# libjxl/jxl-rs

Measured on AMD Instinct MI355X. Metric: megapixels/sec decoded (8K VarDCT d1 reconstruction: dequant+CfL+IDCT+LF smoothing+Gaborish+EPF), higher is better.
Workload: dtype f32

## Files before the change

### jxl_rs_amd/csrc/k_vardct.hip

```cpp
#include <algorithm>
#include <atomic>

#include "k_vardct_common.h"

#ifndef JXLH_NT_COEF
#define JXLH_NT_COEF true
#endif
#ifndef JXLH_NT_K1_STORE
#define JXLH_NT_K1_STORE true
#endif
namespace jxlh {
namespace {

constexpr int kScanGroups = 4;
constexpr int kScanThreads = kScanGroups * kThreads;
template <bool STRIP, bool ENT = false, bool ROUTE = false>
__global__ __launch_bounds__(kScanThreads) void k1_scan(const FrameDev f, const WorkLists wl, const int group_row0,
                                                         int* __restrict__ error_flag,
                                                         const int* __restrict__ group_list, const int ngroups,
                                                         int* __restrict__ next_counts) {
  constexpr int kPairs = (kNumClasses + 1) / 2;
  __shared__ int s_wave_sum[kScanGroups][kWaves];
  __shared__ uint32_t s_wcls[kScanGroups][kWaves][kPairs];
  __shared__ int s_count[kScanGroups][kNumClasses], s_base[kScanGroups][kNumClasses];
  __shared__ int s_route[ROUTE ? kScanGroups : 1];
  __shared__ int s_tmode[kScanGroups][16];
  __shared__ uint64_t s_pref[ENT ? kScanGroups : 1][ENT ? kSlotsPerRun + 1 : 1];
  __shared__ uint64_t s_wpref[ENT ? kScanGroups : 1][kWaves];
  if constexpr (STRIP) {
    if (threadIdx.x < kScanGroups * 16) s_tmode[threadIdx.x / 16][threadIdx.x % 16] = 0;
    if (blockIdx.x == 0)
      for (int i = threadIdx.x; i < f.strip_nflags; i += kScanThreads) f.strip_flags[i] = 0;
    __syncthreads();
  }
  if (blockIdx.x == 0 && threadIdx.x < kCountLines) next_counts[threadIdx.x * kCountPitch] = 0;
  const int sub = threadIdx.x / kThreads, tid = threadIdx.x % kThreads, lane = tid & 63, wave = tid >> 6;
  const int gi = blockIdx.x * kScanGroups + sub;
  const bool live = gi < ngroups;
  const int group = !live ? 0 : group_list ? group_list[gi] : group_row0 * f.xgroups + gi;
  const int bx0 = (group % f.xgroups) * kGroupBlocks, by0 = (group / f.xgroups) * kGroupBlocks;
  const int bw = live ? min(kGroupBlocks, f.xblocks - bx0) : 0, bh = live ? min(kGroupBlocks, f.yblocks - by0) : 0;
  int sizes[4], types[4], rq4[4], local = 0;
  const int by = tid >> 3, bx4 = (tid & 7) * 4;
  const int gby = min(by0 + by, f.yblocks - 1);
  uint8_t raw4[4];
#pragma unroll
  for (int i = 0; i < 4; i++) {
    const size_t at = (size_t)gby * f.xblocks + min(bx0 + bx4 + i, f.xblocks - 1);
    raw4[i] = f.transform_map[at];
    rq4[i] = f.raw_quant[at];
  }
  const int ci = (gby / kColorTileBlocks) * f.cmap_stride + min(bx0 + bx4, f.xblocks - 1) / kColorTileBlocks;
  const uint32_t cc = (uint32_t)(uint8_t)f.ytox[ci] | (uint32_t)(uint8_t)f.ytob[ci] << 8;
  uint32_t cw[3] = {0u, 0u, 0u};
  uint2 run[3] = {make_uint2(0u, 0u), make_uint2(0u, 0u), make_uint2(0u, 0u)};
  bool dense_route = false;
  if constexpr (ENT) {
    if constexpr (ROUTE) {
      dense_route = live && f.group_route[group] != 0;
      if (tid == 0) s_route[sub] = dense_route ? 1 : 0;
    }
    if (live && !dense_route) {
#pragma unroll
      for (int c = 0; c < 3; c++) {
        cw[c] = *reinterpret_cast<const uint32_t*>(f.se_counts + ((size_t)group * 3 + c) * kSlotsPerRun + 4 * tid);
        run[c] = f.se_runs[group * 3 + c];
      }
    }
  }
#pragma unroll
  for (int i = 0; i < 4; i++) {
    const int bx = bx4 + i;
    const uint8_t raw = (bx < bw && by < bh) ? raw4[i] : 0;
    const int type = raw & 127;
    int sz = 0;
    if (raw >= 128) {
      if (type < JXLH_NUM_TRANSFORMS) {
        const int cx = 1 << log2_covered_x_reg(type), cy = 1 << log2_covered_y_reg(type);
        sz = cx * cy;
        if (f.subsampled && sz > 1) atomicExch(error_flag, JXLH_ERR_INVALID_BLOCK_SIZE);
        if (bx + cx > bw || by + cy > bh) {
          atomicExch(error_flag, JXLH_ERR_BLOCK_OUT_OF_BOUNDS);
          sz = 0;
        }
        if constexpr (STRIP) {
          const bool closed = (bx & 3) + cx <= 4 && (by & 3) + cy <= 4 && class_of_type_reg(type) < kClsSpecial;
          if (sz == 0 || f.subsampled) {
            for (int k = 0; k < 16; k++) atomicOr(&s_tmode[sub][k], 1);
          } else if (!closed) {
            for (int ty = by >> 3; ty <= (by + cy - 1) >> 3; ty++)
              for (int tx = bx >> 3; tx <= (bx + cx - 1) >> 3; tx++) atomicOr(&s_tmode[sub][ty * 4 + tx], 1);
          }
        }
      } else {
        atomicExch(error_flag, JXLH_ERR_INVALID_TRANSFORM);
        if constexpr (STRIP)
          for (int k = 0; k < 16; k++) atomicOr(&s_tmode[sub][k], 1);
      }
    }
    sizes[i] = sz;
    types[i] = type;
    local += sz;
  }
  int incl = local;
#pragma unroll
  for (int d = 1; d < 64; d <<= 1) {
    const int n = __shfl_up(incl, d, 64);
    if (lane >= d) incl += n;
  }
  if (lane == 63) s_wave_sum[sub][wave] = incl;
  uint64_t pmine = 0, pincl = 0;
  if constexpr (ENT) {
    auto bytes = [](uint32_t w) { return (uint64_t)((w & 0xffu) + ((w >> 8) & 0xffu) + ((w >> 16) & 0xffu) + (w >> 24)); };
    pmine = bytes(cw[0]) | bytes(cw[1]) << 17 | bytes(cw[2]) << 34;
    pincl = pmine;
#pragma unroll
    for (int d = 1; d < 64; d <<= 1) {
      const uint32_t lo = (uint32_t)__shfl_up((int)(uint32_t)pincl, d, 64), hi = (uint32_t)__shfl_up((int)(uint32_t)(pincl >> 32), d, 64);
      if (lane >= d) pincl += (uint64_t)lo | (uint64_t)hi << 32;
    }
    if (lane == 63) s_wpref[sub][wave] = pincl;
  }
  int slot[4], cls4[4];
  bool strip_tile = false;
  if constexpr (STRIP) {
    __syncthreads();
    strip_tile = s_tmode[sub][(by >> 3) * 4 + (bx4 >> 3)] == 0;
  }
  uint32_t mine[kPairs], excl[kPairs];
#pragma unroll
  for (int w = 0; w < kPairs; w++) mine[w] = 0;
#pragma unroll
  for (int i = 0; i < 4; i++) {
    const int cls = sizes[i] > 0 && !strip_tile ? class_of_type_reg(types[i]) : -1;
    cls4[i] = cls;
    slot[i] = 0;
    const int sh = (cls & 1) * 16;
#pragma unroll
    for (int w = 0; w < kPairs; w++) {
      if ((cls >> 1) == w) {
        slot[i] = (int)((mine[w] >> sh) & 0xffffu);
        mine[w] += 1u << sh;
      }
    }
  }
#pragma unroll
  for (int w = 0; w < kPairs; w++) {
    uint32_t inc = mine[w];
#pragma unroll
    for (int d = 1; d < 64; d <<= 1) {
      const uint32_t n = (uint32_t)__shfl_up((int)inc, d, 64);
      if (lane >= d) inc += n;
    }
    excl[w] = inc - mine[w];
    if (lane == 63) s_wcls[sub][wave][w] = inc;
  }
  __syncthreads();
  if constexpr (ENT) {
    uint64_t base = pincl - pmine;
#pragma unroll
    for (int v = 0; v < kWaves; v++)
      if (v < wave) base += s_wpref[sub][v];
    uint64_t* P = s_pref[sub] + 4 * tid;
#pragma unroll
// ... 226 lines not shown
      }
    };
    EX x = shfl_up(packed, 1);
    if (j == 0) x = 0;
#pragma unroll
    for (int d = 1; d < NS; d <<= 1) {
      const EX y = shfl_up(x, d);
      if (j >= d) x += y;
    }
    if (j < NS) s_excl[b * NS + j] = x;
  }
}
template <class S, class EX>
__device__ __forceinline__ int entry_pos(const EX* __restrict__ s_excl, int b, int ch, uint32_t e, uint32_t r) {
  constexpr int NS = S::N / 64, B = excl_bits<EX>();
  int sidx = 0;
  if constexpr (NS > 1) {
#pragma unroll
    for (int step = NS / 2; step >= 1; step >>= 1) {
      const uint32_t v = (uint32_t)(s_excl[b * NS + sidx + step] >> (B * ch)) & ((1u << B) - 1u);
      if (r >= v) sidx += step;
    }
  }
  return sidx * 64 + (int)(e & 63u);
}
template <class S>
__device__ __forceinline__ void zero_tile(int* __restrict__ ibuf, int lane) {
  constexpr int kWords = S::NB * S::SM;
  if constexpr (kWords % 4 == 0) {
    for (int i = lane * 4; i < kWords; i += 256) *reinterpret_cast<int4*>(ibuf + i) = make_int4(0, 0, 0, 0);
  } else {
    for (int i = lane; i < kWords; i += 64) ibuf[i] = 0;
  }
}

template <class S, int D, class EX, bool HELD = true>
__device__ __forceinline__ void entries_stage_channel(const FrameDev& f, int ch, float* __restrict__ buf,
                                                      const EX* __restrict__ s_excl, int lane, const EntLane<D>& sl,
                                                      const BlockInfo* __restrict__ binfo = nullptr, int nb = 0) {
  int* ibuf = reinterpret_cast<int*>(buf);
  zero_tile<S>(ibuf, lane);
  wave_sync();
  constexpr int LPB = 64 / S::NB;
  const int b = lane / LPB, j = lane % LPB;
  auto add = [&](uint32_t e, uint32_t r) {
    atomicAdd(&ibuf[m_addr<S>(b, entry_pos<S, EX>(s_excl, b, ch, e, r))], (int)(e << 16) >> 22);
  };
  constexpr int DH = HELD ? D : 0;
  uint32_t i0 = 0, i1 = 0;
  if constexpr (HELD) {
    i0 = sl.i0[ch];
    i1 = sl.i1[ch];
  } else if (b < nb) {
    i0 = binfo[b].e0[ch] + j;
    i1 = binfo[b].e0[ch] + binfo[b].en[ch];
  }
#pragma unroll
  for (int k = 0; k < DH; k++)
    if (i0 + k * LPB < i1) add(sl.e[ch][k], (uint32_t)(j + k * LPB));
  constexpr int U = 4;
  uint32_t r = (uint32_t)(j + DH * LPB), i = i0 + DH * LPB;
  while (__any(i < i1)) {
    uint32_t ev[U];
#pragma unroll
    for (int u = 0; u < U; u++) ev[u] = i + u * LPB < i1 ? (uint32_t)f.se_entries[i + u * LPB] : 0u;
#pragma unroll
    for (int u = 0; u < U; u++)
      if (i + u * LPB < i1) add(ev[u], r + u * LPB);
    i += U * LPB;
    r += U * LPB;
  }
  wave_sync();
}

template <int D>
struct EntDirect {
  uint32_t ad[3][D];
};
constexpr uint32_t kNoEntry = 0xffffffffu;
constexpr int kClaimed = (int)0x80000000;

template <class S, int CH, int D>
__device__ __forceinline__ void direct_stage_channel(const FrameDev& f, float* __restrict__ buf, int lane,
                                                     const EntDirect<D>& ed, const float* __restrict__ table, int tsize,
                                                     float sdy, float cc, const AdjTable* __restrict__ adj,
                                                     float (&dyw)[D], uint32_t& ywin) {
  int* ibuf = reinterpret_cast<int*>(buf);
  constexpr int LPB = 64 / S::NB;
  const int b = lane / LPB;
  float w[D];
#pragma unroll
  for (int k = 0; k < D; k++) w[k] = ed.ad[CH][k] != kNoEntry ? table[CH * tsize + (int)(ed.ad[CH][k] & 0xffffu)] : 0.0f;
  zero_tile<S>(ibuf, lane);
  wave_sync();
  int at[D];
#pragma unroll
  for (int k = 0; k < D; k++) {
    at[k] = m_addr<S>(b, (int)(ed.ad[CH][k] & 0x3ffu));
    if (ed.ad[CH][k] != kNoEntry) atomicAdd(&ibuf[at[k]], (int)ed.ad[CH][k] >> 16);
  }
  wave_sync();
  int sum[D];
#pragma unroll
  for (int k = 0; k < D; k++) {
    sum[k] = kClaimed;
    if (ed.ad[CH][k] != kNoEntry) sum[k] = atomicExch(&ibuf[at[k]], kClaimed);
  }
  wave_sync();
  float sd = sdy;
  if constexpr (CH == 0) sd = sdy * f.x_dm;
  if constexpr (CH == 2) sd = sdy * f.b_dm;
#pragma unroll
  for (int k = 0; k < D; k++) {
    if (sum[k] != kClaimed) {
      const int q = sum[k];
      const uint32_t aq = wrapping_abs(q);
      float am = adj->v[CH][min(aq, (uint32_t)kAdjN - 1u)];
      if (aq >= (uint32_t)kAdjN)
        am = __uint_as_float(__float_as_uint(adjust_quant_bias(q, f.quant_biases[CH], f.quant_biases[3])) ^ ((uint32_t)q & 0x80000000u));
      const float a = __uint_as_float(__float_as_uint(am) ^ ((uint32_t)q & 0x80000000u));
      const float mul = w[k] * sd;
      const float v = a * mul;
      if constexpr (CH == 1) {
        dyw[k] = v;
        ywin |= 1u << k;
      }
      buf[at[k]] = v;
    }
  }
  if constexpr (CH != 1) {
    wave_sync();
#pragma unroll
    for (int k = 0; k < D; k++)
      if ((ywin >> k) & 1u) {
        float* t = buf + m_addr<S>(b, (int)(ed.ad[1][k] & 0x3ffu));
        *t = __builtin_fmaf(cc, dyw[k], *t);
      }
  }
  wave_sync();
}

template <class S>
__device__ __forceinline__ int4 tile_q4(const float* __restrict__ buf, int b, int k) {
  const int* ibuf = reinterpret_cast<const int*>(buf);
  if constexpr (S::kWide) {
    return make_int4(ibuf[m_addr<S>(b, k)], ibuf[m_addr<S>(b, k + 1)], ibuf[m_addr<S>(b, k + 2)],
                     ibuf[m_addr<S>(b, k + 3)]);
  } else {
    return *reinterpret_cast<const int4*>(ibuf + m_addr<S>(b, k));
  }
}

template <class S, bool PREFETCH, int SPARSE, bool SUB = false, int CLS = 0, bool INLINE_FB = false, bool LISTED = false,
          class EX = uint32_t>
__device__ __forceinline__ int run_dct_class(const FrameDev& f, const WorkItem* __restrict__ items,
                                             const EntryItem* __restrict__ eitems, int count, int type,
                                             float* __restrict__ buf, BlockInfo* __restrict__ binfo_base,
                                             EX* __restrict__ s_excl, float* __restrict__ s_lf, int gwave,
                                             int nwaves, int lane, const AdjTable* __restrict__ adj,
                                             uint32_t* __restrict__ wl_fallback = nullptr,
                                             int* __restrict__ fallback_count = nullptr, float* __restrict__ s_dy = nullptr,
                                             uint32_t fb_first_flag = 0, uint32_t* __restrict__ wl_fb_any = nullptr,
                                             int* fb_rank = nullptr) {
  constexpr int NCH = S::E / 4;
  const int q = quant_table_for_type(type);
  const float* __restrict__ table = f.tables + f.table_offset[q];
  const int tsize = quant_table_size(q);
  const int nbatches = (count + S::NB - 1) / S::NB;
  constexpr int kFbChunk = 16;
  struct BatchIter {
    int bi;
    unsigned long long mask;
    bool pre;
  };
  const int it_wave = gwave % kWaves, it_wg = gwave / kWaves, it_nwg = nwaves / kWaves;
  auto iter_next = [&](BatchIter& st) -> int {
    if constexpr (!LISTED) {
      const int b = st.bi;
      st.bi += nwaves;
      return b < nbatches ? b : -1;
    } else {
      for (;;) {
        while (st.mask) {
          const int bit = __builtin_ctzll(st.mask);
          st.mask &= st.mask - 1;
          const int chunk = st.pre ? st.bi + (bit >> 4) * it_nwg : st.bi;
          if ((*fb_rank)++ % kWaves == it_wave) return chunk * kFbChunk + (bit & 15);
        }
        st.bi += st.pre ? 4 * it_nwg : it_nwg;
        st.pre = false;
        if (st.bi * kFbChunk >= nbatches) return -1;
        const int idx = st.bi * kFbChunk + lane;
        st.mask = __ballot(lane < kFbChunk && idx < nbatches && wl_fallback[idx] == (uint32_t)f.fb_epoch);
      }
    }
  };
  static_assert(kFbChunk == 16, "the prefetched mask holds four 16-batch chunks");
  BatchIter iter = {LISTED ? it_wg : gwave, LISTED ? __ballot(fb_first_flag == (uint32_t)f.fb_epoch && fb_first_flag != 0) : 0ull, LISTED};
  constexpr bool kPF = PREFETCH && SPARSE != 3;
  float4 tw[kPF ? 3 : 1][NCH];
  if constexpr (kPF) {
#pragma unroll
    for (int c = 0; c < 3; c++)
#pragma unroll
      for (int j = 0; j < NCH; j++)
        tw[c][j] = *reinterpret_cast<const float4*>(table + c * tsize + ((j * 64 + lane) * 4) % S::N);
  }
  constexpr bool kChain = SPARSE >= 2;
#ifndef JXLH_ITEM_PREFETCH
#define JXLH_ITEM_PREFETCH 1
#endif
  constexpr bool kNextItem = kChain && !LISTED && (JXLH_ITEM_PREFETCH == 2 || (JXLH_ITEM_PREFETCH == 1 && PREFETCH));
  constexpr int kLfPerBlock = 3 * (S::R / 8) * (S::C / 8), kLfIters = (S::NB * kLfPerBlock + 63) / 64;
  WorkItem it_next = {};
  EntryItem ei_next = {};
  if constexpr (kNextItem) {
    if (gwave < nbatches && lane < min(S::NB, count - gwave * S::NB)) {
      it_next = items[gwave * S::NB + lane];
      ei_next = eitems[gwave * S::NB + lane];
    }
  }
  int n_dense_pass = 0;
  bool flagged_any = false;
  for (int batch = iter_next(iter); batch >= 0; batch = iter_next(iter)) {
    const int nb = min(S::NB, count - batch * S::NB);
    if constexpr (LISTED) n_dense_pass++;
    BlockInfo* __restrict__ binfo = binfo_base;
    bool direct_ok = true;
    if constexpr (kChain) {
      WorkItem it = it_next;
      EntryItem ei = ei_next;
      if constexpr (kNextItem) {
        const int nxt = batch + nwaves;
        if (nxt < nbatches && lane < min(S::NB, count - nxt * S::NB)) {
          it_next = items[nxt * S::NB + lane];
          ei_next = eitems[nxt * S::NB + lane];
        }
      } else if (lane < nb) {
        it = items[batch * S::NB + lane];
        ei = eitems[batch * S::NB + lane];
      }
      bool item_ok = true;
      if (lane < nb) {
        decode_item(f, it, &binfo[lane]);
#pragma unroll
        for (int c = 0; c < 3; c++) binfo[lane].e0[c] = ei.e0[c];
        binfo[lane].en[0] = ei.nxy & 0xffffu;
        binfo[lane].en[1] = ei.nxy >> 16;
        binfo[lane].en[2] = it.group >> 16;
        if constexpr (SPARSE == 3) {
          const float sdy = binfo[lane].sdy;
          item_ok = sdy > 0.0f && sdy < __builtin_inff() &&
                    max(max(ei.nxy & 0xffffu, ei.nxy >> 16), it.group >> 16) <= (uint32_t)(ent_depth<S>() * (64 / S::NB));
        }
      }
      if constexpr (SPARSE == 3 && !INLINE_FB) {
        if (!__all(item_ok)) {
          if (lane == 0) {
            wl_fallback[batch] = (uint32_t)f.fb_epoch;
            if (!flagged_any) wl_fb_any[(gwave % kFbAny) * kFbAnyPitch] = (uint32_t)f.fb_epoch;
          }
          flagged_any = true;
          continue;
        }
      } else {
        direct_ok = __all(item_ok);
      }
    } else if (lane < nb) {
      const WorkItem it = items[batch * S::NB + lane];
      decode_item(f, it, &binfo[lane]);
    }
    wave_sync();
    SparseLane sl;
    constexpr int D = ent_depth<S>();
    EntLane<D> el;
    if constexpr (SPARSE == 1) {
      sparse_ranges<S>(f, binfo, nb, lane, sl);
      sparse_first<S>(f, sl);
    } else if constexpr (SPARSE >= 2) {
      entries_begin<S, D, EX>(f, binfo, s_excl, nb, lane, el);
    }
    if constexpr (kChain) {
      float lfv[kLfIters];
#pragma unroll
      for (int i = 0; i < kLfIters; i++) {
        const int idx = i * 64 + lane, b = idx / kLfPerBlock, rem = idx % kLfPerBlock;
        const int c = rem / ((S::R / 8) * (S::C / 8)), yx = rem % ((S::R / 8) * (S::C / 8));
        const int y = yx / (S::C / 8), x = yx % (S::C / 8);
        lfv[i] = 0.0f;
        if (b < nb) {
          const float* __restrict__ lp = c == 0 ? f.lf[0] : c == 1 ? f.lf[1] : f.lf[2];
          lfv[i] = lp[binfo[b].lf_off[c] + y * f.xblocks + x];
        }
      }
#pragma unroll
      for (int i = 0; i < kLfIters; i++)
        if (i * 64 + lane < S::NB * kLfPerBlock) s_lf[i * 64 + lane] = lfv[i];
    }
    auto transform_channel = [&](auto ch_tag) {
      constexpr int CH = decltype(ch_tag)::value;
      const float* __restrict__ lfp = f.lf[CH];
      float* __restrict__ plane = f.planes[CH];
      const PixLayout lay = pix_layout(f);
      const int xblocks = f.xblocks;
      idct_batch<S>(
          buf, nb, lane,
          [&](int b, int y, int x) {
            if constexpr (kChain) return s_lf[b * kLfPerBlock + (CH * (S::R / 8) + y) * (S::C / 8) + x];
            else return lfp[binfo[b].lf_off[CH] + y * xblocks + x];
          },
          [&](int b, int x, int yb, const float(&v)[8]) {
            if (SUB && binfo[b].px_off[CH] == f.scrap_off) return;
            float* dst = plane + binfo[b].px_off[CH] + lay.xoff(x) + yb * lay.ystep_blk;
            if (lay.tiled) {
              gstore_f4<JXLH_NT_K1_STORE>(dst, make_float4(v[0], v[1], v[2], v[3]));
              gstore_f4<JXLH_NT_K1_STORE>(dst + 32, make_float4(v[4], v[5], v[6], v[7]));
            } else {
#pragma unroll
              for (int i = 0; i < 8; i++) dst[i * lay.ystep8] = v[i];
            }
          });
    };
    using TagX = std::integral_constant<int, 0>;
    using TagY = std::integral_constant<int, 1>;
    using TagB = std::integral_constant<int, 2>;
    auto generic_batch = [&](auto mode_tag) {
      constexpr int GM = decltype(mode_tag)::value;
      int4 qv[kPF ? 3 : 1][NCH];
      if constexpr (kPF && !GM) {
#pragma unroll
        for (int c = 0; c < 3; c++)
#pragma unroll
          for (int j = 0; j < NCH; j++) {
            const int fl = (j * 64 + lane) * 4;
            const int b = fl / S::N, k = fl % S::N;
            qv[c][j] = make_int4(0, 0, 0, 0);
            if (b < nb && (!SUB || binfo[b].px_off[c] != f.scrap_off))
              qv[c][j] = gload_i4<JXLH_NT_COEF>(f.coeffs + binfo[b].coef_off + c * kGroupArea + k);
          }
      }
      constexpr bool kRecomputeY = !GM && !PREFETCH && S::E > 16;
      constexpr bool kDyLds = GM == 2 && SPARSE == 2 && S::E > 16;
      float dy[kRecomputeY || kDyLds ? 4 : S::E];
      auto stage_channel = [&](auto ch_tag) {
        constexpr int CH = decltype(ch_tag)::value;
        if constexpr (GM == 1) sparse_stage_channel<S>(f, CH, buf, lane, sl);
        if constexpr (GM == 2) entries_stage_channel<S, D, EX, SPARSE == 2>(f, CH, buf, s_excl, lane, el, binfo, nb);
#pragma unroll
        for (int j = 0; j < NCH; j++) {
          const int fl = (j * 64 + lane) * 4;
          const int b = fl / S::N, k = fl % S::N;
          float4 v = make_float4(0.f, 0.f, 0.f, 0.f);
          float d4[4];
          if constexpr (kRecomputeY) {
            d4[0] = d4[1] = d4[2] = d4[3] = 0.0f;
          } else if constexpr (kDyLds) {
            d4[0] = d4[1] = d4[2] = d4[3] = 0.0f;
            if constexpr (CH != 1) {
              const float4 t = *reinterpret_cast<const float4*>(s_dy + (j * 64 + lane) * 4);
              d4[0] = t.x;
              d4[1] = t.y;
              d4[2] = t.z;
              d4[3] = t.w;
            }
          } else {
            d4[0] = dy[j * 4];
            d4[1] = dy[j * 4 + 1];
            d4[2] = dy[j * 4 + 2];
            d4[3] = dy[j * 4 + 3];
          }
          if (b < nb) {
            const BlockInfo bi = binfo[b];
            int4 qq;
            float4 tt;
            if constexpr (GM != 0) {
              qq = tile_q4<S>(buf, b, k);
              if constexpr (kPF) tt = tw[CH][j];
              else tt = *reinterpret_cast<const float4*>(table + CH * tsize + k);
            } else if constexpr (kPF) {
              qq = qv[CH][j];
              tt = tw[CH][j];
            } else {
              qq = gload_i4<JXLH_NT_COEF>(f.coeffs + bi.coef_off + CH * kGroupArea + k);
              tt = *reinterpret_cast<const float4*>(table + CH * tsize + k);
              if constexpr (kRecomputeY && CH != 1) {
                const int4 qy = gload_i4<false>(f.coeffs + bi.coef_off + kGroupArea + k);
                const float4 ty = *reinterpret_cast<const float4*>(table + tsize + k);
                (void)dequant4t<1>(f, qy, ty, bi, adj, d4);
              }
            }
            v = dequant4t<CH>(f, qq, tt, bi, adj, d4);
          }
          if constexpr (CH == 1 && kDyLds) {
            *reinterpret_cast<float4*>(s_dy + (j * 64 + lane) * 4) = make_float4(d4[0], d4[1], d4[2], d4[3]);
          } else if constexpr (CH == 1 && !kRecomputeY) {
            dy[j * 4] = d4[0];
            dy[j * 4 + 1] = d4[1];
            dy[j * 4 + 2] = d4[2];
            dy[j * 4 + 3] = d4[3];
          }
          stage4<S>(buf, b, k, v);
        }
        wave_sync();
      };
      stage_channel(TagY{});
      transform_channel(TagY{});
      stage_channel(TagX{});
      transform_channel(TagX{});
      stage_channel(TagB{});
      transform_channel(TagB{});
    };
    if constexpr (SPARSE == 3) {
      constexpr int LPB = 64 / S::NB;
      const int b = lane / LPB, j = lane % LPB;
      float sdy = 0.0f, xcc = 0.0f, bcc = 0.0f;
      if (b < nb) {
        sdy = binfo[b].sdy;
        xcc = binfo[b].x_cc;
        bcc = binfo[b].b_cc;
      }
      if constexpr (INLINE_FB) {
        if (!direct_ok) {
          static_assert(S::N == 64, "the inline fallback has no slot prefixes: one-slot varblocks only");
          generic_batch(std::integral_constant<int, 2>{});
          n_dense_pass++;
          wave_sync();
          continue;
        }
      }
      wave_sync();
      EntDirect<D> ed;
#pragma unroll
      for (int c = 0; c < 3; c++)
#pragma unroll
        for (int k = 0; k < D; k++) {
          ed.ad[c][k] = kNoEntry;
          if (el.i0[c] + k * LPB < el.i1[c]) {
            const uint32_t e = el.e[c][k];
            ed.ad[c][k] = (uint32_t)entry_pos<S, EX>(s_excl, b, c, e, (uint32_t)(j + k * LPB)) | (uint32_t)((int)(e << 16) >> 22) << 16;
          }
        }
      float dyw[D];
      uint32_t ywin = 0;
#pragma unroll
      for (int k = 0; k < D; k++) dyw[k] = 0.0f;
      direct_stage_channel<S, 1, D>(f, buf, lane, ed, table, tsize, sdy, 0.0f, adj, dyw, ywin);
      transform_channel(TagY{});
      direct_stage_channel<S, 0, D>(f, buf, lane, ed, table, tsize, sdy, xcc, adj, dyw, ywin);
      transform_channel(TagX{});
      direct_stage_channel<S, 2, D>(f, buf, lane, ed, table, tsize, sdy, bcc, adj, dyw, ywin);
      transform_channel(TagB{});
    } else {
      generic_batch(std::integral_constant<int, SPARSE>{});
    }
  }
  if (f.k1_stats && (LISTED || INLINE_FB) && n_dense_pass && lane == 0) atomicAdd(fallback_count, n_dense_pass);
  return nbatches;
}

__device__ __forceinline__ int rotate_wave(int gw, int used, int nw) {
  const int r = (gw - used % nw) % nw;
  return r < 0 ? r + nw : r;
}

template <class S>
struct ShapeTag {
  using type = S;
};
using S8x8 = Shape<8, 8>;
using S16x16 = Shape<16, 16>;
using S32x32 = Shape<32, 32>;
using S16x8 = Shape<16, 8>;
using S8x16 = Shape<8, 16>;
using S32x8 = Shape<32, 8, 4>;
using S8x32 = Shape<8, 32>;
using S32x16 = Shape<32, 16>;
using S16x32 = Shape<16, 32>;

constexpr int kTileA = S8x8::kTile;
constexpr int kTileC = cmax(cmax(cmax(S32x8::kTile, S8x32::kTile), cmax(S32x16::kTile, S16x32::kTile)),
                            S32x32::kTile);

template <int SPARSE, bool SUB = false, bool INLINE = false>
#ifndef JXLH_K1_INLINE_WPE
#define JXLH_K1_INLINE_WPE 1
#endif
__global__ __launch_bounds__(kThreads, SPARSE == 3 ? (INLINE ? JXLH_K1_INLINE_WPE : 6) : 1) void k1_dct8(const FrameDev f, const WorkLists wl) {
  __shared__ __attribute__((aligned(16))) float s_buf[kWaves * kTileA];
  __shared__ BlockInfo s_binfo[kWaves][S8x8::NB];
  __shared__ AdjTable s_adj;
  build_adj_table(f, &s_adj, threadIdx.x, kThreads);
  const int lane = threadIdx.x & 63, wave = threadIdx.x >> 6;
  __shared__ float s_lf[SPARSE >= 2 ? kWaves : 1][S8x8::NB * 3];
  static_assert(!INLINE || SPARSE == 3, "the inline fallback belongs to the direct form");
  run_dct_class<S8x8, true, SPARSE, SUB, kClsDct8, INLINE>(f, wl.items[kClsDct8], wl.eitems[kClsDct8], wl.counts[(kClsDct8) * kCountPitch], 0,
                                                   s_buf + wave * kTileA, s_binfo[wave], (uint32_t*)nullptr, s_lf[SPARSE >= 2 ? wave : 0],
                                                   blockIdx.x * kWaves + wave, gridDim.x * kWaves, lane, &s_adj,
                                                   wl.fallback[kClsDct8], wl.counts + (kCntFallback0 + kClsDct8) * kCountPitch, nullptr, 0u,
                                                   wl.fb_any);
}

constexpr int kExclWords = 40;
#ifndef JXLH_K1_MERGED
#define JXLH_K1_MERGED 0
#endif
#ifndef JXLH_K1_DIRECT_WPE
#define JXLH_K1_DIRECT_WPE 3
#endif
constexpr int kDyWords = 32 * 64;
template <int SPARSE, bool FB = false, bool ALL = false>
__global__ __launch_bounds__(kThreads, SPARSE == 3 ? JXLH_K1_DIRECT_WPE : SPARSE == 2 ? 2 : 3) void k1_dct16_32(const FrameDev f, const WorkLists wl) {
  static_assert(!FB || SPARSE == 2, "the fallback launch runs the dense dequantisation pass of the entries form");
  static_assert(!ALL || SPARSE == 0, "one launch for every DCT class: dense slabs only");
  uint32_t fb_pre[kClsSpecial] = {};
  uint32_t fb_live = 0;
  if constexpr (FB) {
    const uint32_t summary = wl.fb_any[(threadIdx.x & (kFbAny - 1)) * kFbAnyPitch];
    constexpr int kOrder[kClsSpecial] = {kClsDct32x32, kClsDct32x16, kClsDct16x32, kClsDct32x8, kClsDct8x32,
                                         kClsDct16x16, kClsDct16x8,  kClsDct8x16,  kClsDct8};
    constexpr int kNb[kClsSpecial] = {S32x32::NB, S32x16::NB, S16x32::NB, S32x8::NB, S8x32::NB, S16x16::NB, S16x8::NB, S8x16::NB, S8x8::NB};
    const int grid = (int)gridDim.x, l = threadIdx.x & 63;
    int nbat[kClsSpecial];
#pragma unroll
    for (int k = 0; k < kClsSpecial; k++) nbat[k] = (wl.counts[kOrder[k] * kCountPitch] + kNb[k] - 1) / kNb[k];
    if (!__any(summary == (uint32_t)f.fb_epoch)) return;
    int used = 0;
#pragma unroll
    for (int k = 0; k < kClsSpecial; k++) {
      const int nch = (nbat[k] + 15) / 16, fc = rotate_wave((int)blockIdx.x, used, grid), idx = (fc + (l >> 4) * grid) * 16 + (l & 15);
      fb_pre[k] = idx < nbat[k] ? wl.fallback[kOrder[k]][idx] : 0u;
      if (fc + 4 * grid < nch) fb_live |= 1u << k;
      used += nch;
    }
#pragma unroll
    for (int k = 0; k < kClsSpecial; k++)
      if (__any(fb_pre[k] == (uint32_t)f.fb_epoch)) fb_live |= 1u << k;
    if (!fb_live) return;
  }
  __shared__ __attribute__((aligned(16))) float s_buf[kWaves * kTileC];
  __shared__ BlockInfo s_binfo[kWaves][8];
  using EX = std::conditional_t<SPARSE == 2, uint64_t, uint32_t>;
  __shared__ EX s_excl[SPARSE >= 2 ? kWaves : 1][kExclWords];
  __shared__ AdjTable s_adj;
  build_adj_table(f, &s_adj, threadIdx.x, kThreads);
  const int lane = threadIdx.x & 63, wave = threadIdx.x >> 6;
  float* buf = s_buf + wave * kTileC;
  EX* ex = s_excl[SPARSE >= 2 ? wave : 0];
  __shared__ float s_lfs[SPARSE >= 2 ? kWaves : 1][96];
  float* lfs = s_lfs[SPARSE >= 2 ? wave : 0];
  __shared__ __attribute__((aligned(16))) float s_dyb[SPARSE == 2 ? kWaves * kDyWords : 4];
  float* sdy = SPARSE == 2 ? s_dyb + wave * kDyWords : nullptr;
  const int gw = blockIdx.x * kWaves + wave, nw = gridDim.x * kWaves;
  auto cnt = [&](int cls) { return wl.counts[cls * kCountPitch]; };
  int used = 0, fb_rank = 0;
  auto run = [&](auto shape_tag, auto pf_tag, auto cls_tag, int type, int fb_k = 0) {
    using S = typename decltype(shape_tag)::type;
    constexpr bool PF = decltype(pf_tag)::value;
    constexpr int CLS = decltype(cls_tag)::value;
    if constexpr (FB) {
      if (!((fb_live >> fb_k) & 1u)) {
        used += ((cnt(CLS) + S::NB - 1) / S::NB + 15) / 16;
        return;
      }
    }
    const int nbat = run_dct_class<S, PF, SPARSE, false, CLS, false, FB>(
        f, wl.items[CLS], wl.eitems[CLS], cnt(CLS), type, buf, s_binfo[wave], ex, lfs,
        FB ? rotate_wave((int)blockIdx.x, used, (int)gridDim.x) * kWaves + wave : rotate_wave(gw, used, nw), nw, lane, &s_adj,
        wl.fallback[CLS], wl.counts + (kCntFallback0 + CLS) * kCountPitch, sdy, FB ? fb_pre[fb_k] : 0u, wl.fb_any, &fb_rank);
    used += FB ? (nbat + 15) / 16 : nbat;
  };
  run(ShapeTag<S32x32>{}, std::false_type{}, std::integral_constant<int, kClsDct32x32>{}, 5, 0);
  run(ShapeTag<S32x16>{}, std::false_type{}, std::integral_constant<int, kClsDct32x16>{}, 10, 1);
  run(ShapeTag<S16x32>{}, std::false_type{}, std::integral_constant<int, kClsDct16x32>{}, 11, 2);
  run(ShapeTag<S32x8>{}, std::false_type{}, std::integral_constant<int, kClsDct32x8>{}, 8, 3);
  run(ShapeTag<S8x32>{}, std::false_type{}, std::integral_constant<int, kClsDct8x32>{}, 9, 4);
  run(ShapeTag<S16x16>{}, std::true_type{}, std::integral_constant<int, kClsDct16x16>{}, 4, 5);
  run(ShapeTag<S16x8>{}, std::true_type{}, std::integral_constant<int, kClsDct16x8>{}, 6, 6);
  run(ShapeTag<S8x16>{}, std::true_type{}, std::integral_constant<int, kClsDct8x16>{}, 7, 7);
  if constexpr (FB) run(ShapeTag<S8x8>{}, std::true_type{}, std::integral_constant<int, kClsDct8>{}, 0, 8);
  if constexpr (ALL) run(ShapeTag<S8x8>{}, std::true_type{}, std::integral_constant<int, kClsDct8>{}, 0);
}

constexpr int kSpecWaves = 2;
constexpr int kSpecThreads = kSpecWaves * 64;
constexpr int kSpecChunk = 512;
constexpr int kSpecBins = 9;
constexpr int kSpecBlk = 21;
constexpr int kSpecIters = (kSpecBlk * 16 + 63) / 64;
__device__ __forceinline__ int special_bin(int type) {
  return type <= 3 ? type - 1 : type - 9;
}

template <int TYPE>
__device__ __forceinline__ void special_8x8_inplace(float* __restrict__ row, const float* __restrict__ afv_basis = kAfvBasisDev) {
  float c[64], o[64];
#pragma unroll
  for (int i = 0; i < 64; i++) c[i] = row[i];
  special_8x8_t<TYPE>(c, o, afv_basis);
#pragma unroll
  for (int i = 0; i < 64; i++) row[i] = o[i];
}

template <int BIN0, int BIN1>
__global__ __launch_bounds__(kSpecThreads) void k1_special(const FrameDev f, const WorkLists wl) {
  __shared__ float s_tile[kSpecWaves][64 * kSpecPitch];
  __shared__ BlockInfo s_binfo[kSpecWaves][kSpecBlk];
  __shared__ int s_idx[kSpecWaves][kSpecChunk];
  __shared__ AdjTable s_adj;
  __shared__ float s_afv[BIN1 > 5 ? 256 : 1];
  if constexpr (BIN1 > 5)
    for (int i = threadIdx.x; i < 256; i += kSpecThreads) s_afv[i] = kAfvBasisDev[i];
  build_adj_table(f, &s_adj, threadIdx.x, kSpecThreads);
  const int lane = threadIdx.x & 63, wave = threadIdx.x >> 6;
  const WorkItem* __restrict__ items = wl.items[kClsSpecial];
  const int count = wl.counts[(kClsSpecial) * kCountPitch];
  float* tile = s_tile[wave];
  BlockInfo* binfo = s_binfo[wave];
  int* mine = s_idx[wave];
  constexpr int kBins = BIN1 - BIN0;
  const int npairs = ((count + kSpecChunk - 1) / kSpecChunk) * kBins;
  for (int pair = blockIdx.x * kSpecWaves + wave; pair < npairs; pair += gridDim.x * kSpecWaves) {
    const int chunk = pair / kBins, bin = BIN0 + pair % kBins;
    int nmine = 0;
    uint32_t packed[kSpecChunk / 64];
#pragma unroll
    for (int i = 0; i < kSpecChunk / 64; i++) {
      const int idx = chunk * kSpecChunk + i * 64 + lane;
      packed[i] = items[min(idx, max(count - 1, 0))].packed;
    }
#pragma unroll
    for (int i = 0; i < kSpecChunk / 64; i++) {
      const int idx = chunk * kSpecChunk + i * 64 + lane;
      const bool m = idx < count && special_bin((int)(packed[i] >> 20) & 31) == bin;
      const unsigned long long mask = __ballot(m);
      if (m) mine[nmine + __popcll(mask & ((1ull << lane) - 1ull))] = idx;
      nmine += __popcll(mask);
    }
    wave_sync();
    constexpr int kBinType[kSpecBins] = {1, 2, 3, 12, 13, 14, 15, 16, 17};
    int bin_type = kBinType[0];
#pragma unroll
    for (int i = 1; i < kSpecBins; i++) bin_type = bin == i ? kBinType[i] : bin_type;
    const float* __restrict__ bin_table = f.tables + f.table_offset[quant_table_for_type(bin_type)];
    const int k0 = (lane & 15) * 4;
    for (int b0 = 0; b0 < nmine; b0 += kSpecBlk) {
      const int nb = min(kSpecBlk, nmine - b0);
      if (lane < nb) {
        const WorkItem it = items[mine[b0 + lane]];
        decode_item(f, it, &binfo[lane]);
      }
      wave_sync();
      float dy[4 * kSpecIters];
      auto stage_channel = [&](auto ch_tag) {
        constexpr int CH = decltype(ch_tag)::value;
        const float4 tv = *reinterpret_cast<const float4*>(bin_table + CH * 64 + k0);
        int4 qv[kSpecIters];
        float b_sdy[kSpecIters], b_xcc[kSpecIters], b_bcc[kSpecIters];
#pragma unroll
        for (int j = 0; j < kSpecIters; j++) {
          const int b = min(j * 4 + (lane >> 4), nb - 1);
          const BlockInfo* bp = &binfo[b];
          b_sdy[j] = bp->sdy;
          b_xcc[j] = bp->x_cc;
          b_bcc[j] = bp->b_cc;
          qv[j] = gload_i4<JXLH_NT_COEF>(f.coeffs + bp->coef_off + CH * kGroupArea + k0);
        }
#pragma unroll
        for (int j = 0; j < kSpecIters; j++) {
          const int b = j * 4 + (lane >> 4);
          float d4[4] = {dy[j * 4], dy[j * 4 + 1], dy[j * 4 + 2], dy[j * 4 + 3]};
          BlockInfo bi;
          bi.sdy = b_sdy[j];
          bi.x_cc = b_xcc[j];
          bi.b_cc = b_bcc[j];
          const float4 v = dequant4t<CH>(f, qv[j], tv, bi, &s_adj, d4);
          if constexpr (CH == 1) {
            dy[j * 4] = d4[0];
            dy[j * 4 + 1] = d4[1];
            dy[j * 4 + 2] = d4[2];
            dy[j * 4 + 3] = d4[3];
          }
          if (b < nb) {
            float* dst = tile + (CH * kSpecBlk + b) * kSpecPitch + k0;
            dst[0] = v.x;
            dst[1] = v.y;
            dst[2] = v.z;
            dst[3] = v.w;
          }
        }
      };
      stage_channel(std::integral_constant<int, 1>{});
      stage_channel(std::integral_constant<int, 0>{});
      stage_channel(std::integral_constant<int, 2>{});
      const int tch = lane / kSpecBlk, tb = lane % kSpecBlk;
      const bool on = tch < 3 && tb < nb;
      const float lf0 = f.lf[min(tch, 2)][binfo[min(tb, nb - 1)].lf_off[min(tch, 2)]];
      wave_sync();
      if (on) {
        float* row = tile + lane * kSpecPitch;
        row[0] = lf0;
        auto in_range = [](int b) { return b >= BIN0 && b < BIN1; };
        if (in_range(0) && bin == 0) special_8x8_inplace<1>(row);
        if (in_range(1) && bin == 1) special_8x8_inplace<2>(row);
        if (in_range(2) && bin == 2) special_8x8_inplace<3>(row);
        if (in_range(3) && bin == 3) special_8x8_inplace<12>(row);
        if (in_range(4) && bin == 4) special_8x8_inplace<13>(row);
        if (in_range(5) && bin == 5) special_8x8_inplace<14>(row, s_afv);
        if (in_range(6) && bin == 6) special_8x8_inplace<15>(row, s_afv);
        if (in_range(7) && bin == 7) special_8x8_inplace<16>(row, s_afv);
        if (in_range(8) && bin == 8) special_8x8_inplace<17>(row, s_afv);
      }
      wave_sync();
#pragma unroll
      for (int ch = 0; ch < 3; ch++) {
        float* __restrict__ plane = f.planes[ch];
        float4 ov[kSpecIters];
        int oo[kSpecIters];
#pragma unroll
        for (int j = 0; j < kSpecIters; j++) {
          const int b = min(j * 4 + (lane >> 4), nb - 1), p = k0;
          const int px = binfo[b].px_off[ch];
// ... 194 lines not shown
```

### jxl_rs_amd/csrc/varblock_core.h

```cpp
#pragma once
#include "dct_device.h"
#include "jxlh_internal.h"

namespace jxlh {

__device__ __forceinline__ void wave_sync() {
  __builtin_amdgcn_fence(__ATOMIC_RELEASE, "wavefront");
  __builtin_amdgcn_wave_barrier();
  __builtin_amdgcn_fence(__ATOMIC_ACQUIRE, "wavefront");
}

constexpr int cmin(int a, int b) { return a < b ? a : b; }
constexpr int cmax(int a, int b) { return a < b ? b : a; }

template <int R_, int C_, int NB_ = 64 / (R_ < C_ ? R_ : C_)>
struct Shape {
  static constexpr int R = R_, C = C_;
  static constexpr bool kWide = R < C;
  static constexpr int kMin = cmin(R, C), kMax = cmax(R, C);
  static constexpr int NB = NB_;
  static constexpr int N = R * C;
  static constexpr int E = NB * N / 64;
  static constexpr int LM = kWide ? R + 1 : R;
  static constexpr int SM_raw = C * LM;
  static constexpr int SM = SM_raw + ((R % 32) - (SM_raw % 32) + 32) % 32;
  static constexpr int LT = C + 4;
  static constexpr int ST_raw = R * LT;
  static constexpr int ST = ST_raw + ((C % 32) - (ST_raw % 32) + 32) % 32;
  static constexpr int I1 = (NB * R + 63) / 64;
  static constexpr int I2 = (NB * C + 63) / 64;
  static constexpr int kTile = NB * cmax(SM, ST);
  static_assert(SM % 4 == 0 || kWide, "float4 staging needs 16-byte aligned blocks");
  static_assert(ST % 4 == 0 && LT % 4 == 0, "float4 row writes");
};

template <class S>
__device__ __forceinline__ int m_addr(int b, int k) {
  if constexpr (S::kWide) {
    const int v = k / S::C, u = k % S::C;
    return b * S::SM + u * S::LM + v;
  } else {
    return b * S::SM + k;
  }
}

template <int CY, int CX>
__device__ __forceinline__ void llf_from_lf(float (&a)[CY * CX]) {
  constexpr bool kF = cmin(CY, CX) > 4;
  if constexpr (CY == 1 && CX == 1) {
    return;
  } else if constexpr (CY < CX) {
#pragma unroll
    for (int y = 0; y < CY; y++) {
      float t[CX];
#pragma unroll
      for (int x = 0; x < CX; x++) t[x] = a[y * CX + x];
      rdct1d<CX, kF>(t);
#pragma unroll
      for (int x = 0; x < CX; x++) a[y * CX + x] = t[x];
    }
#pragma unroll
    for (int x = 0; x < CX; x++) {
      float t[CY];
#pragma unroll
      for (int y = 0; y < CY; y++) t[y] = a[y * CX + x];
      rdct1d<CY, kF>(t);
#pragma unroll
      for (int y = 0; y < CY; y++) a[y * CX + x] = t[y];
    }
  } else {
    float o[CY * CX];
#pragma unroll
    for (int x = 0; x < CX; x++) {
      float t[CY];
#pragma unroll
      for (int y = 0; y < CY; y++) t[y] = a[y * CX + x];
      rdct1d<CY, kF>(t);
#pragma unroll
      for (int y = 0; y < CY; y++) a[y * CX + x] = t[y];
    }
#pragma unroll
    for (int v = 0; v < CY; v++) {
      float t[CX];
#pragma unroll
      for (int x = 0; x < CX; x++) t[x] = a[v * CX + x];
      rdct1d<CX, kF>(t);
#pragma unroll
      for (int u = 0; u < CX; u++) o[u * CY + v] = t[u];
    }
#pragma unroll
    for (int i = 0; i < CY * CX; i++) a[i] = o[i];
  }
}

template <class S, class LfLoad, class Store>
__device__ __forceinline__ void idct_batch(float* __restrict__ buf, int nb, int lane, LfLoad lf_load,
                                           Store store) {
  constexpr int R = S::R, C = S::C;
  constexpr int CY = R / 8, CX = C / 8;
  if (lane < nb) {
    float a[CY * CX];
#pragma unroll
    for (int y = 0; y < CY; y++)
#pragma unroll
      for (int x = 0; x < CX; x++) a[y * CX + x] = lf_load(lane, y, x);
    llf_from_lf<CY, CX>(a);
    constexpr int MN = cmin(CY, CX), MX = cmax(CY, CX);
#pragma unroll
    for (int r = 0; r < MN; r++)
#pragma unroll
      for (int q = 0; q < MX; q++) buf[m_addr<S>(lane, r * S::kMax + q)] = a[r * MX + q];
  }
  wave_sync();
  float p1[S::I1][C];
#pragma unroll
  for (int it = 0; it < S::I1; it++) {
    const int t = it * 64 + lane;
    const int b = min(t / R, S::NB - 1), v = t % R;
    const float* src = buf + b * S::SM + v;
#pragma unroll
    for (int u = 0; u < C; u++) p1[it][u] = src[u * S::LM];
    idct1d<C, true>(p1[it]);
  }
  wave_sync();
#pragma unroll
  for (int it = 0; it < S::I1; it++) {
    const int t = it * 64 + lane;
    const int b = t / R, v = t % R;
    if (b < S::NB) {
      float4* dst = reinterpret_cast<float4*>(buf + b * S::ST + v * S::LT);
#pragma unroll
      for (int x = 0; x < C; x += 4) dst[x / 4] = make_float4(p1[it][x], p1[it][x + 1], p1[it][x + 2], p1[it][x + 3]);
    }
  }
  wave_sync();
#pragma unroll
  for (int it = 0; it < S::I2; it++) {
    const int t = it * 64 + lane;
    const int b = t / C, x = t % C;
    float col[R];
    const float* src = buf + min(b, S::NB - 1) * S::ST + x;
#pragma unroll
    for (int v = 0; v < R; v++) col[v] = src[v * S::LT];
    idct1d<R, true>(col);
    if (b < nb) {
#pragma unroll
      for (int yb = 0; yb < R / 8; yb++) {
        const float v8[8] = {col[yb * 8],     col[yb * 8 + 1], col[yb * 8 + 2], col[yb * 8 + 3],
                             col[yb * 8 + 4], col[yb * 8 + 5], col[yb * 8 + 6], col[yb * 8 + 7]};
        store(b, x, yb, v8);
      }
    }
  }
  wave_sync();
}

constexpr int kSpecPitch = 65;
constexpr int kSpecNB = 32;

__constant__ float kAfvBasisDev[256] = {
#include "afv_basis.inc"
};

template <int R, int C>
__device__ __forceinline__ void idct2d_small(float (&d)[R * C]) {
  constexpr bool kF = cmin(R, C) > 4;
  if constexpr (R < C) {
#pragma unroll
    for (int v = 0; v < R; v++) {
      float t[C];
#pragma unroll
      for (int u = 0; u < C; u++) t[u] = d[v * C + u];
      idct1d<C, kF>(t);
#pragma unroll
      for (int u = 0; u < C; u++) d[v * C + u] = t[u];
    }
#pragma unroll
    for (int x = 0; x < C; x++) {
      float t[R];
#pragma unroll
      for (int v = 0; v < R; v++) t[v] = d[v * C + x];
      idct1d<R, kF>(t);
#pragma unroll
      for (int v = 0; v < R; v++) d[v * C + x] = t[v];
    }
  } else {
    float o[R * C];
#pragma unroll
    for (int v = 0; v < R; v++) {
      float t[C];
#pragma unroll
      for (int u = 0; u < C; u++) t[u] = d[u * R + v];
      idct1d<C, kF>(t);
#pragma unroll
      for (int x = 0; x < C; x++) o[v * C + x] = t[x];
    }
#pragma unroll
    for (int x = 0; x < C; x++) {
      float t[R];
#pragma unroll
      for (int v = 0; v < R; v++) t[v] = o[v * C + x];
      idct1d<R, kF>(t);
#pragma unroll
      for (int y = 0; y < R; y++) d[y * C + x] = t[y];
    }
  }
}

template <int S>
__device__ __forceinline__ void idct2_top_block(const float* in, float* out) {
  constexpr int num = S / 2;
#pragma unroll
  for (int y = 0; y < num; y++) {
#pragma unroll
    for (int x = 0; x < num; x++) {
      const float c00 = in[y * 8 + x];
      const float c01 = in[y * 8 + num + x];
      const float c10 = in[(y + num) * 8 + x];
      const float c11 = in[(y + num) * 8 + num + x];
      out[y * 2 * 8 + x * 2] = c00 + c01 + c10 + c11;
      out[y * 2 * 8 + x * 2 + 1] = c00 + c01 - c10 - c11;
      out[(y * 2 + 1) * 8 + x * 2] = c00 - c01 + c10 - c11;
      out[(y * 2 + 1) * 8 + x * 2 + 1] = c00 - c01 - c10 + c11;
    }
  }
}

template <int TYPE>
__device__ __forceinline__ void special_8x8_t(float* __restrict__ c, float* __restrict__ o,
                                              const float* __restrict__ afv_basis = kAfvBasisDev) {
  if constexpr (TYPE == 1) {
    const float b00 = c[0], b01 = c[1], b10 = c[8], b11 = c[9];
    const float dcs[4] = {b00 + b01 + b10 + b11, b00 + b01 - b10 - b11, b00 - b01 + b10 - b11,
                          b00 - b01 - b10 + b11};
#pragma unroll
    for (int y = 0; y < 2; y++) {
#pragma unroll
      for (int x = 0; x < 2; x++) {
        float residual_sum = 0.0f;
#pragma unroll
        for (int iy = 0; iy < 4; iy++)
#pragma unroll
          for (int ix = 0; ix < 4; ix++) {
            if (ix == 0 && iy == 0) continue;
            residual_sum += c[(y + iy * 2) * 8 + x + ix * 2];
          }
        const float pivot = dcs[y * 2 + x] - residual_sum * (1.0f / 16.0f);
#pragma unroll
        for (int iy = 0; iy < 4; iy++)
#pragma unroll
          for (int ix = 0; ix < 4; ix++) {
            if (ix == 1 && iy == 1) continue;
            o[(y * 4 + iy) * 8 + x * 4 + ix] = c[(y + iy * 2) * 8 + x + ix * 2] + pivot;
          }
        o[(4 * y + 1) * 8 + 4 * x + 1] = pivot;
        o[y * 4 * 8 + x * 4] = c[(y + 2) * 8 + x + 2] + pivot;
      }
    }
  } else if constexpr (TYPE == 2) {
    idct2_top_block<2>(c, o);
#pragma unroll
    for (int i = 0; i < 64; i++) {
      const int y = i / 8, x = i % 8;
      if (y >= 2 || x >= 2) o[i] = c[i];
    }
    idct2_top_block<4>(o, c);
#pragma unroll
    for (int i = 0; i < 64; i++) {
      const int y = i / 8, x = i % 8;
      if (y >= 4 || x >= 4) c[i] = o[i];
    }
    idct2_top_block<8>(c, o);
  } else if constexpr (TYPE == 3) {
    const float b00 = c[0], b01 = c[1], b10 = c[8], b11 = c[9];
    const float dcs[4] = {b00 + b01 + b10 + b11, b00 + b01 - b10 - b11, b00 - b01 + b10 - b11,
                          b00 - b01 - b10 + b11};
#pragma unroll
    for (int y = 0; y < 2; y++)
#pragma unroll
      for (int x = 0; x < 2; x++) {
        float blk[16];
#pragma unroll
        for (int iy = 0; iy < 4; iy++)
#pragma unroll
          for (int ix = 0; ix < 4; ix++)
            blk[iy * 4 + ix] = (ix == 0 && iy == 0) ? dcs[y * 2 + x] : c[(y + iy * 2) * 8 + x + ix * 2];
        idct2d_small<4, 4>(blk);
#pragma unroll
        for (int iy = 0; iy < 4; iy++)
#pragma unroll
          for (int ix = 0; ix < 4; ix++) o[(y * 4 + iy) * 8 + x * 4 + ix] = blk[iy * 4 + ix];
      }
  } else if constexpr (TYPE == 13) {
    const float dcs[2] = {c[0] + c[8], c[0] - c[8]};
#pragma unroll
    for (int x = 0; x < 2; x++) {
      float blk[32];
#pragma unroll
      for (int iy = 0; iy < 4; iy++)
#pragma unroll
        for (int ix = 0; ix < 8; ix++)
          blk[iy * 8 + ix] = (ix == 0 && iy == 0) ? dcs[x] : c[(x + iy * 2) * 8 + ix];
      idct2d_small<8, 4>(blk);
#pragma unroll
      for (int iy = 0; iy < 8; iy++)
#pragma unroll
        for (int ix = 0; ix < 4; ix++) o[iy * 8 + x * 4 + ix] = blk[iy * 4 + ix];
    }
  } else if constexpr (TYPE == 12) {
// ... 95 lines not shown
```

Measured before the change: 101,500.

## Pipeline dense k1 coefficient loads into LDS across channels via async global_load_lds

Adds a pipelined path for dense (non-sparse, non-prefetch) varblock classes. Once a channel's column pass has read its data out of the LDS tile, the next channel's coefficients (or the next batch's Y channel) are issued as asynchronous global-to-LDS loads, so they overlap the remaining IDCT work. It also packs Y quantized coefficients into 8 bits in shared memory for CfL reuse by the X and B channels when they fit, falling back to a global reload otherwise. The cost is extra shared memory per wave, more register pressure from holding whole column arrays, and more complex wave synchronisation.

```diff
diff --git a/jxl_rs_amd/csrc/k_vardct.hip b/jxl_rs_amd/csrc/k_vardct.hip
--- a/jxl_rs_amd/csrc/k_vardct.hip
+++ b/jxl_rs_amd/csrc/k_vardct.hip
@@ -9,7 +9,18 @@
 #ifndef JXLH_NT_K1_STORE
 #define JXLH_NT_K1_STORE true
 #endif
+#ifndef JXLH_K1_DENSE_PIPE
+#define JXLH_K1_DENSE_PIPE 1
+#endif
+#ifndef EXP_NOPACK
+#define EXP_NOPACK 0
+#endif
+#ifndef EXP_ONLY
+#define EXP_ONLY -1
+#endif
 namespace jxlh {
+typedef __attribute__((address_space(1))) const void* k1_gptr_t;
+typedef __attribute__((address_space(3))) void* k1_lptr_t;
 namespace {
 
 constexpr int kScanGroups = 4;
@@ -542,7 +553,7 @@
 }
 
 template <class S, bool PREFETCH, int SPARSE, bool SUB = false, int CLS = 0, bool INLINE_FB = false, bool LISTED = false,
-          class EX = uint32_t>
+          bool PIPE = false, class EX = uint32_t>
 __device__ __forceinline__ int run_dct_class(const FrameDev& f, const WorkItem* __restrict__ items,
                                              const EntryItem* __restrict__ eitems, int count, int type,
                                              float* __restrict__ buf, BlockInfo* __restrict__ binfo_base,
@@ -551,7 +562,8 @@
                                              uint32_t* __restrict__ wl_fallback = nullptr,
                                              int* __restrict__ fallback_count = nullptr, float* __restrict__ s_dy = nullptr,
                                              uint32_t fb_first_flag = 0, uint32_t* __restrict__ wl_fb_any = nullptr,
-                                             int* fb_rank = nullptr) {
+                                             int* fb_rank = nullptr, uint32_t* __restrict__ s_ypk = nullptr) {
+  static_assert(!PIPE || (SPARSE == 0 && !PREFETCH && !SUB && !LISTED), "the pipelined body: dense slabs, 16..32-point classes");
   constexpr int NCH = S::E / 4;
   const int q = quant_table_for_type(type);
   const float* __restrict__ table = f.tables + f.table_offset[q];
@@ -612,8 +624,32 @@
   }
   int n_dense_pass = 0;
   bool flagged_any = false;
+  static_assert(!PIPE || (S::N % 256 == 0 && S::E * 64 <= S::kTile), "pieces of whole varblocks, a channel fits the tile");
+  WorkItem pit = {};
+  auto request = [&](auto ch_tag, auto coef_of, int nbr) {
+    constexpr int CH = decltype(ch_tag)::value;
+#pragma unroll
+    for (int j = 0; j < NCH; j++) {
+      const int b = j * 256 / S::N, k = (j * 256) % S::N + lane * 4;
+      if (b < nbr)
+        __builtin_amdgcn_global_load_lds((k1_gptr_t)(f.coeffs + coef_of(b) + CH * kGroupArea + k), (k1_lptr_t)(buf + j * 256), 16, 0,
+                                         JXLH_NT_COEF ? 2 : 0);
+    }
+  };
+  auto item_coef = [&](int b) {
+    const uint32_t g = __shfl(pit.group, b), pk = __shfl(pit.packed, b);
+    return (int)(g & 0xffffu) * 3 * kGroupArea + (int)((pk >> 10) & 1023u) * 64;
+  };
+  if constexpr (PIPE) {
+    if (gwave < nbatches) {
+      const int nb0 = min(S::NB, count - gwave * S::NB);
+      if (lane < nb0) pit = items[gwave * S::NB + lane];
+      request(std::integral_constant<int, 1>{}, item_coef, nb0);
+    }
+  }
   for (int batch = iter_next(iter); batch >= 0; batch = iter_next(iter)) {
     const int nb = min(S::NB, count - batch * S::NB);
+    int nb_next = 0;
     if constexpr (LISTED) n_dense_pass++;
     BlockInfo* __restrict__ binfo = binfo_base;
     bool direct_ok = true;
@@ -656,6 +692,11 @@
       } else {
         direct_ok = __all(item_ok);
       }
+    } else if constexpr (PIPE) {
+      if (lane < nb) decode_item(f, pit, &binfo[lane]);
+      const int nxt = batch + nwaves;
+      if (nxt < nbatches) nb_next = min(S::NB, count - nxt * S::NB);
+      if (lane < nb_next) pit = items[nxt * S::NB + lane];
     } else if (lane < nb) {
       const WorkItem it = items[batch * S::NB + lane];
       decode_item(f, it, &binfo[lane]);
@@ -710,6 +751,26 @@
               for (int i = 0; i < 8; i++) dst[i * lay.ystep8] = v[i];
             }
           });
+    };
+    auto transform_channel_pipe = [&](auto ch_tag, auto tile_free) {
+      constexpr int CH = decltype(ch_tag)::value;
+      const float* __restrict__ lfp = f.lf[CH];
+      float* __restrict__ plane = f.planes[CH];
+      const PixLayout lay = pix_layout(f);
+      const int xblocks = f.xblocks;
+      idct_batch_tile_free<S>(
+          buf, nb, lane, [&](int b, int y, int x) { return lfp[binfo[b].lf_off[CH] + y * xblocks + x]; },
+          [&](int b, int x, int yb, const float(&v)[8]) {
+            float* dst = plane + binfo[b].px_off[CH] + lay.xoff(x) + yb * lay.ystep_blk;
+            if (lay.tiled) {
+              gstore_f4<JXLH_NT_K1_STORE>(dst, make_float4(v[0], v[1], v[2], v[3]));
+              gstore_f4<JXLH_NT_K1_STORE>(dst + 32, make_float4(v[4], v[5], v[6], v[7]));
+            } else {
+#pragma unroll
+              for (int i = 0; i < 8; i++) dst[i * lay.ystep8] = v[i];
+            }
+          },
+          tile_free);
     };
     using TagX = std::integral_constant<int, 0>;
     using TagY = std::integral_constant<int, 1>;
@@ -793,6 +854,84 @@
         }
         wave_sync();
       };
+      if constexpr (PIPE && !GM) {
+        constexpr bool kPackY = S::E > 16 && !EXP_NOPACK;
+        bool y_packed = false;
+        auto pipe_stage = [&](auto ch_tag, auto packed_tag) {
+          constexpr int CH = decltype(ch_tag)::value;
+          constexpr bool kFromPack = decltype(packed_tag)::value;
+          uint32_t wide = 0;
+          const int* __restrict__ raw = reinterpret_cast<const int*>(buf);
+          static_assert(S::kWide || S::SM == S::N, "in-place conversion");
+          int4 qw[S::kWide ? NCH : 1];
+          if constexpr (S::kWide) {
+#pragma unroll
+            for (int j = 0; j < NCH; j++) qw[j] = *reinterpret_cast<const int4*>(raw + j * 256 + lane * 4);
+            wave_sync();
+          }
+#pragma unroll
+          for (int j = 0; j < NCH; j++) {
+            const int b = j * 256 / S::N, k = (j * 256) % S::N + lane * 4;
+            float4 v = make_float4(0.f, 0.f, 0.f, 0.f);
+            float d4[4];
+            if constexpr (kPackY) {
+              d4[0] = d4[1] = d4[2] = d4[3] = 0.0f;
+            } else {
+              d4[0] = dy[j * 4];
+              d4[1] = dy[j * 4 + 1];
+              d4[2] = dy[j * 4 + 2];
+              d4[3] = dy[j * 4 + 3];
+            }
+            int4 qq = make_int4(0, 0, 0, 0);
+            if (b < nb) {
+              const BlockInfo bi = binfo[b];
+              if constexpr (S::kWide) qq = qw[j];
+              else qq = *reinterpret_cast<const int4*>(raw + j * 256 + lane * 4);
+              const float4 tt = *reinterpret_cast<const float4*>(table + CH * tsize + k);
+              if constexpr (kPackY && CH != 1) {
+                int4 qy;
+                if constexpr (kFromPack) {
+                  const uint32_t w = s_ypk[j * 64 + lane];
+                  qy = make_int4((int)(w << 24) >> 24, (int)(w << 16) >> 24, (int)(w << 8) >> 24, (int)w >> 24);
+                } else {
+                  qy = gload_i4<false>(f.coeffs + bi.coef_off + kGroupArea + k);
+                }
+                const float4 ty = *reinterpret_cast<const float4*>(table + tsize + k);
+                (void)dequant4t<1>(f, qy, ty, bi, adj, d4);
+              }
+              v = dequant4t<CH>(f, qq, tt, bi, adj, d4);
+            }
+            if constexpr (CH == 1 && kPackY) {
+              s_ypk[j * 64 + lane] = ((uint32_t)qq.x & 0xffu) | ((uint32_t)qq.y & 0xffu) << 8 | ((uint32_t)qq.z & 0xffu) << 16 | (uint32_t)qq.w << 24;
+              wide |= ((uint32_t)qq.x + 128u) | ((uint32_t)qq.y + 128u) | ((uint32_t)qq.z + 128u) | ((uint32_t)qq.w + 128u);
+            } else if constexpr (CH == 1) {
+              dy[j * 4] = d4[0];
+              dy[j * 4 + 1] = d4[1];
+              dy[j * 4 + 2] = d4[2];
+              dy[j * 4 + 3] = d4[3];
+            }
+            stage4<S>(buf, b, k, v);
+          }
+          if constexpr (CH == 1 && kPackY) y_packed = !__any(wide >= 256u);
+          wave_sync();
+        };
+        auto pipe_stage_xb = [&](auto ch_tag) {
+          if constexpr (kPackY) {
+            if (y_packed) pipe_stage(ch_tag, std::true_type{});
+            else pipe_stage(ch_tag, std::false_type{});
+          } else {
+            pipe_stage(ch_tag, std::false_type{});
+          }
+        };
+        auto binfo_coef = [&](int b) { return binfo[b].coef_off; };
+        pipe_stage(TagY{}, std::false_type{});
+        transform_channel_pipe(TagY{}, [&] { request(TagX{}, binfo_coef, nb); });
+        pipe_stage_xb(TagX{});
+        transform_channel_pipe(TagX{}, [&] { request(TagB{}, binfo_coef, nb); });
+        pipe_stage_xb(TagB{});
+        transform_channel_pipe(TagB{}, [&] { request(TagY{}, item_coef, nb_next); });
+        return;
+      }
       stage_channel(TagY{});
       transform_channel(TagY{});
       stage_channel(TagX{});
@@ -940,6 +1079,8 @@
   float* lfs = s_lfs[SPARSE >= 2 ? wave : 0];
   __shared__ __attribute__((aligned(16))) float s_dyb[SPARSE == 2 ? kWaves * kDyWords : 4];
   float* sdy = SPARSE == 2 ? s_dyb + wave * kDyWords : nullptr;
+  constexpr bool kPipe = JXLH_K1_DENSE_PIPE && SPARSE == 0 && !ALL;
+  __shared__ uint32_t s_ypk[kPipe ? kWaves * 512 : 4];
   const int gw = blockIdx.x * kWaves + wave, nw = gridDim.x * kWaves;
   auto cnt = [&](int cls) { return wl.counts[cls * kCountPitch]; };
   int used = 0, fb_rank = 0;
@@ -947,16 +1088,17 @@
     using S = typename decltype(shape_tag)::type;
     constexpr bool PF = decltype(pf_tag)::value;
     constexpr int CLS = decltype(cls_tag)::value;
+    if constexpr (EXP_ONLY >= 0 && SPARSE == 0 && !ALL) { if (fb_k != EXP_ONLY) return; }
     if constexpr (FB) {
       if (!((fb_live >> fb_k) & 1u)) {
         used += ((cnt(CLS) + S::NB - 1) / S::NB + 15) / 16;
         return;
       }
     }
-    const int nbat = run_dct_class<S, PF, SPARSE, false, CLS, false, FB>(
+    const int nbat = run_dct_class<S, PF, SPARSE, false, CLS, false, FB, kPipe && !PF>(
         f, wl.items[CLS], wl.eitems[CLS], cnt(CLS), type, buf, s_binfo[wave], ex, lfs,
         FB ? rotate_wave((int)blockIdx.x, used, (int)gridDim.x) * kWaves + wave : rotate_wave(gw, used, nw), nw, lane, &s_adj,
-        wl.fallback[CLS], wl.counts + (kCntFallback0 + CLS) * kCountPitch, sdy, FB ? fb_pre[fb_k] : 0u, wl.fb_any, &fb_rank);
+        wl.fallback[CLS], wl.counts + (kCntFallback0 + CLS) * kCountPitch, sdy, FB ? fb_pre[fb_k] : 0u, wl.fb_any, &fb_rank, kPipe ? s_ypk + wave * 512 : nullptr);
     used += FB ? (nbat + 15) / 16 : nbat;
   };
   run(ShapeTag<S32x32>{}, std::false_type{}, std::integral_constant<int, kClsDct32x32>{}, 5, 0);
diff --git a/jxl_rs_amd/csrc/varblock_core.h b/jxl_rs_amd/csrc/varblock_core.h
--- a/jxl_rs_amd/csrc/varblock_core.h
+++ b/jxl_rs_amd/csrc/varblock_core.h
@@ -155,6 +155,75 @@
   wave_sync();
 }
 
+template <class S, class LfLoad, class Store, class Hook>
+__device__ __forceinline__ void idct_batch_tile_free(float* __restrict__ buf, int nb, int lane, LfLoad lf_load,
+                                                     Store store, Hook tile_free) {
+  constexpr int R = S::R, C = S::C;
+  constexpr int CY = R / 8, CX = C / 8;
+  if (lane < nb) {
+    float a[CY * CX];
+#pragma unroll
+    for (int y = 0; y < CY; y++)
+#pragma unroll
+      for (int x = 0; x < CX; x++) a[y * CX + x] = lf_load(lane, y, x);
+    llf_from_lf<CY, CX>(a);
+    constexpr int MN = cmin(CY, CX), MX = cmax(CY, CX);
+#pragma unroll
+    for (int r = 0; r < MN; r++)
+#pragma unroll
+      for (int q = 0; q < MX; q++) buf[m_addr<S>(lane, r * S::kMax + q)] = a[r * MX + q];
+  }
+  wave_sync();
+  float p1[S::I1][C];
+#pragma unroll
+  for (int it = 0; it < S::I1; it++) {
+    const int t = it * 64 + lane;
+    const int b = min(t / R, S::NB - 1), v = t % R;
+    const float* src = buf + b * S::SM + v;
+#pragma unroll
+    for (int u = 0; u < C; u++) p1[it][u] = src[u * S::LM];
+    idct1d<C, true>(p1[it]);
+  }
+  wave_sync();
+#pragma unroll
+  for (int it = 0; it < S::I1; it++) {
+    const int t = it * 64 + lane;
+    const int b = t / R, v = t % R;
+    if (b < S::NB) {
+      float4* dst = reinterpret_cast<float4*>(buf + b * S::ST + v * S::LT);
+#pragma unroll
+      for (int x = 0; x < C; x += 4) dst[x / 4] = make_float4(p1[it][x], p1[it][x + 1], p1[it][x + 2], p1[it][x + 3]);
+    }
+  }
+  wave_sync();
+  float col[S::I2][R];
+#pragma unroll
+  for (int it = 0; it < S::I2; it++) {
+    const int t = it * 64 + lane;
+    const float* src = buf + min(t / C, S::NB - 1) * S::ST + t % C;
+#pragma unroll
+    for (int v = 0; v < R; v++) col[it][v] = src[v * S::LT];
+  }
+  wave_sync();
+  __asm__ volatile("s_waitcnt lgkmcnt(0)" ::: "memory");
+  tile_free();
+#pragma unroll
+  for (int it = 0; it < S::I2; it++) {
+    const int t = it * 64 + lane;
+    const int b = t / C, x = t % C;
+    idct1d<R, true>(col[it]);
+    if (b < nb) {
+#pragma unroll
+      for (int yb = 0; yb < R / 8; yb++) {
+        const float v8[8] = {col[it][yb * 8],     col[it][yb * 8 + 1], col[it][yb * 8 + 2], col[it][yb * 8 + 3],
+                             col[it][yb * 8 + 4], col[it][yb * 8 + 5], col[it][yb * 8 + 6], col[it][yb * 8 + 7]};
+        store(b, x, yb, v8);
+      }
+    }
+  }
+  wave_sync();
+}
+
 constexpr int kSpecPitch = 65;
 constexpr int kSpecNB = 32;
 
```

Result: no change. 99240, median of 2 (-2.2%).
